# jc-bao/gym-xarm

Measured on AMD Instinct MI355X. Metric: env steps/sec (whole node), XarmPDPickAndPlace-v0, higher is better.
Workload: dtype f32

## Files before the change

### gym_xarm_amd/build.py

```python
import os
import shutil
import subprocess
import sys

HERE = os.path.dirname(os.path.abspath(__file__))
CSRC = os.path.join(HERE, "csrc")
LIB = os.path.join(CSRC, "libxarm_hip.so")
UNITS = ["xarm_hip.hip", "xarm_k_pnp.hip", "xarm_k_pnp_coop.hip", "xarm_k_reach.hip", "xarm_k_handover.hip", "xarm_k_handover_coop.hip",
         "xarm_k_handover2.hip", "xarm_k_stack.hip", "xarm_k_rearrange.hip", "xarm_k_render.hip", "xarm_k_her.hip", "xarm_k_norm.hip"]
HEADERS = ["xarm_dev.h", "xarm_core.h", "xarm7_pd_model.h", "xarm_reach_core.h", "xarm7_reach_model.h", "xarm_handover_core.h", "xarm_handover2_core.h",
           "xarm_stack_core.h", "xarm_rearrange_core.h", "xarm_coop_core.h", "xarm_reach_coop_core.h", "xarm_handover_coop_core.h", "xarm_render_core.h",
           "xarm_render_model.h", "xarm_her_core.h", "xarm_norm_core.h"]
SOURCES = UNITS + HEADERS
UNIT_FLAGS = {"xarm_k_handover_coop.hip": ["-ffp-contract=on", "-DXC_SWEEP_COPY"], "xarm_k_norm.hip": ["-ffp-contract=off"]}
_SCHED = [] if os.environ.get("XARM_SCHED", "ilp") == "default" else ["-mllvm", "-amdgpu-sched-strategy=iterative-ilp"]
HIPCC_FLAGS = ["--offload-arch=gfx950", "-O3", "-std=c++17", "-fPIC", "-Wno-unused-value", "-fno-slp-vectorize"] + _SCHED

def find_hipcc():
    for c in (os.environ.get("HIPCC"), shutil.which("hipcc"), "/opt/rocm/bin/hipcc"):
        if c and os.path.exists(c):
            return c
    raise RuntimeError("hipcc not found (need ROCm); set HIPCC=/path/to/hipcc")


def stale():
    if not os.path.exists(LIB):
        return True
    deps = [os.path.join(CSRC, s) for s in SOURCES] + [os.path.join(os.path.dirname(HERE), "include", "xarm_hip.h")]
    t = os.path.getmtime(LIB)
    return any(os.path.getmtime(d) > t for d in deps if os.path.exists(d))


def _compile(args):
    cmd, verbose = args
    if verbose:
        print(" ".join(cmd), flush=True)
    subprocess.check_call(cmd)


def build(force=False, verbose=True, extra_flags=(), lib=LIB, jobs=None):
    from concurrent.futures import ThreadPoolExecutor
    for g in ("gen_model_header.py", "gen_render_header.py"):
        gen = os.path.join(os.path.dirname(HERE), "tools", g)
        if os.path.exists(gen):
            subprocess.check_call([sys.executable, gen], stdout=subprocess.DEVNULL)
    if not force and lib == LIB and not stale():
        return lib
    hipcc = find_hipcc()
    objdir = os.path.join(CSRC, "build" if lib == LIB else "build_" + os.path.splitext(os.path.basename(lib))[0])
    os.makedirs(objdir, exist_ok=True)
    objs, jobs_l = [], []
    for u in UNITS:
        o = os.path.join(objdir, os.path.splitext(u)[0] + ".o")
        objs.append(o)
        jobs_l.append(([hipcc] + HIPCC_FLAGS + UNIT_FLAGS.get(u, []) + list(extra_flags) + ["-c", "-o", o, os.path.join(CSRC, u)], verbose))
    with ThreadPoolExecutor(jobs or min(len(UNITS), os.cpu_count() or 1)) as ex:
        list(ex.map(_compile, jobs_l))
    _compile(([hipcc, "--offload-arch=gfx950", "-shared", "-fPIC", "-o", lib] + objs, verbose))
    return lib


def build_example(verbose=True):
    root = os.path.dirname(HERE)
    src, out = os.path.join(root, "examples", "abi_step_loop.c"), os.path.join(root, "examples", "abi_step_loop")
    if not os.path.exists(src):
        return None
    if os.path.exists(out) and os.path.getmtime(out) >= max(os.path.getmtime(src), os.path.getmtime(os.path.join(root, "include", "xarm_hip.h"))):
        return out
    rocm = os.environ.get("ROCM_PATH", "/opt/rocm")
    cmd = ["gcc", "-O2", "-std=c11", "-I", os.path.join(root, "include"), "-I", os.path.join(rocm, "include"), src,
           "-L", CSRC, "-lxarm_hip", "-L", os.path.join(rocm, "lib"), "-lamdhip64",
           "-Wl,-rpath,$ORIGIN/../gym_xarm_amd/csrc", "-Wl,-rpath," + os.path.join(rocm, "lib"), "-o", out]
    if verbose:
        print(" ".join(cmd), flush=True)
    subprocess.check_call(cmd)
    return out


if __name__ == "__main__":
    build(force="--force" in sys.argv)
    print(LIB)
```

### gym_xarm_amd/csrc/xarm_coop_core.h

```cpp
#pragma once
#include "xarm_core.h"

namespace xc {
using xk::V3; using xk::mk; using xk::dot; using xk::cross; using xk::symmul; using xk::tri; using xk::symi;
using xk::EnvState; using xk::EnvCfg; using xk::NTS; using xk::NP; using xk::clampT; using xk::xabs; using xk::xsqrt;
using xk::LDS_S; using xk::LDS_T;

constexpr int GL = 16;
constexpr int NT = 3 * NTS;
constexpr int NA1 = 14;
constexpr int NF = 3 * NP;
constexpr int NLA = 7;
constexpr int C0_T = 0, C0_F = NT, C0_N = NT + NF;
constexpr int C1_A = 0, C1_L = NA1, C1_F = NA1 + NLA, C1_N = NA1 + NLA + NF;
constexpr int C2_T = 0, C2_A = NT, C2_L = NT + NA1, C2_F = NT + NA1 + NLA, C2_N = NT + NA1 + NLA + NF;

#if defined(__HIPCC__) && !defined(XARM_HOST_BUILD)
constexpr int LVN = 1;
struct Grp { int l; };
XARM_HD int lane_of(const Grp &G, int) { return G.l; }
template <int CTRL> XARM_HD float dpp(float x) {
    return __builtin_bit_cast(float, __builtin_amdgcn_update_dpp(0, __builtin_bit_cast(int, x), CTRL, 0xf, 0xf, true));
}
#else
// ... 59 lines not shown
#endif
template <int L, typename T> XARM_HD T lv_get(LV<T> x) { return lv_bcast<L>(x).v[0]; }
#if defined(__HIPCC__) && !defined(XARM_HOST_BUILD)
XARM_HD LV<float> lv_suffix_sum(LV<float> x) {
    XC_NO_CONTRACT
    float s = x.v[0];
    s += dpp<0x101>(s);
    s += dpp<0x102>(s);
    s += dpp<0x104>(s);
    s += dpp<0x108>(s);
    LV<float> r; r.v[0] = s; return r;
}
#else
template <typename T> XARM_HD LV<T> lv_suffix_sum(LV<T> x) {
    T a[GL], b[GL];
    for (int i = 0; i < GL; i++) a[i] = x.v[i];
    for (int sh = 1; sh < GL; sh *= 2) {
        for (int i = 0; i < GL; i++) b[i] = a[i] + (i + sh < GL ? a[i + sh] : (T)0);
        for (int i = 0; i < GL; i++) a[i] = b[i];
    }
    LV<T> r; for (int i = 0; i < GL; i++) r.v[i] = a[i]; return r;
}
#endif

#if defined(__HIPCC__) && !defined(XARM_HOST_BUILD)
template <typename T> struct LV2 { xk::xf2 v; };
XARM_HD LV2<float> lv2_make(LV<float> x, LV<float> y) { LV2<float> r; r.v.x = x.v[0]; r.v.y = y.v[0]; return r; }
XARM_HD LV<float> lv2_x(LV2<float> a) { LV<float> r; r.v[0] = a.v.x; return r; }
XARM_HD LV<float> lv2_y(LV2<float> a) { LV<float> r; r.v[0] = a.v.y; return r; }
XARM_HD LV2<float> lv2_fma(LV2<float> a, LV2<float> b, LV2<float> c) { LV2<float> r; r.v = __builtin_elementwise_fma(a.v, b.v, c.v); return r; }
XARM_HD LV2<float> lv2_sub(LV2<float> a, LV2<float> b) { XC_NO_CONTRACT LV2<float> r; r.v = a.v - b.v; return r; }
XARM_HD LV2<float> lv2_mul(LV2<float> a, LV2<float> b) { XC_NO_CONTRACT LV2<float> r; r.v = a.v * b.v; return r; }
template <int L> XARM_HD void lv2_commit(const Grp &G, LV2<float> &dst, LV2<float> src) { dst.v = G.l == L ? src.v : dst.v; }
template <int L> XARM_HD LV2<float> lv2_bcast(LV2<float> x) {
    LV2<float> r;
    const long long in = __builtin_bit_cast(long long, x.v);
    const long long out = __builtin_amdgcn_update_dpp(0ll, in, 0x150 + L, 0xf, 0xf, true);
    r.v = __builtin_bit_cast(xk::xf2, out);
    return r;
}
#else
template <typename T> struct LV2 { LV<T> x, y; };
template <typename T> XARM_HD LV2<T> lv2_make(LV<T> x, LV<T> y) { LV2<T> r; r.x = x; r.y = y; return r; }
template <typename T> XARM_HD LV<T> lv2_x(LV2<T> a) { return a.x; }
template <typename T> XARM_HD LV<T> lv2_y(LV2<T> a) { return a.y; }
template <typename T> XARM_HD LV2<T> lv2_fma(LV2<T> a, LV2<T> b, LV2<T> c) { return lv2_make(lv_fma(a.x, b.x, c.x), lv_fma(a.y, b.y, c.y)); }
template <typename T> XARM_HD LV2<T> lv2_sub(LV2<T> a, LV2<T> b) { return lv2_make(lv_sub(a.x, b.x), lv_sub(a.y, b.y)); }
template <typename T> XARM_HD LV2<T> lv2_mul(LV2<T> a, LV2<T> b) { return lv2_make(lv_mul(a.x, b.x), lv_mul(a.y, b.y)); }
template <int L, typename T> XARM_HD void lv2_commit(const Grp &G, LV2<T> &dst, LV2<T> src) { lv_commit<L>(G, dst.x, src.x); lv_commit<L>(G, dst.y, src.y); }
template <int L, typename T> XARM_HD LV2<T> lv2_bcast(LV2<T> x) { return lv2_make(lv_bcast<L>(x.x), lv_bcast<L>(x.y)); }
#endif

template <typename T> XARM_HD T sel3(int k, T a, T b, T c) { return k == 0 ? a : (k == 1 ? b : c); }
template <typename T> XARM_HD T sel4(int k, T a, T b, T c, T d) { return k == 0 ? a : (k == 1 ? b : (k == 2 ? c : d)); }
template <typename T> XARM_HD V3<T> selv3(int k, V3<T> a, V3<T> b, V3<T> c) { return mk<T>(sel3(k, a.x, b.x, c.x), sel3(k, a.y, b.y, c.y), sel3(k, a.z, b.z, c.z)); }
template <typename T> XARM_HD V3<T> selv4(int k, V3<T> a, V3<T> b, V3<T> c, V3<T> d) {
    return mk<T>(sel4(k, a.x, b.x, c.x, d.x), sel4(k, a.y, b.y, c.y, d.y), sel4(k, a.z, b.z, c.z, d.z));
}

template <typename T> struct Setup {
    T Minv[45], dq[9];
    V3<T> hc1;
    V3<T> cb, vb, wb;
    T Iinv[6];
    V3<T> tr[NTS];
    T tvt[NTS], tl0[NTS];
    int tid[NTS];
    T m_vt[9], la_vt[7], la_sg[7], lf_vt[2][2], g_vt;
    LV<T> lpp[3], lpn[3], lpt1[3], lpvt, lpl0;
    bool pact[NP];
    bool pad_any, la_any;
    T pad_cfm, mu_p;
};

enum { R_J0 = 0,
       R_J1 = 6,
       R_J2A = 15,
       R_J2B = 24,
       R_J3 = 30,
       R_G = 37,
       R_L0 = 41,
       R_LO1 = 45, R_HI1 = 46,
       R_CFM = 47,
       R_N = 48 };

template <typename T> XARM_HD V3<T> tdir(int a) { return mk<T>(a == 2 ? (T)1 : (T)0, a == 1 ? (T)-1 : (T)0, a == 0 ? (T)1 : (T)0); }

template <typename T, typename Scene = xk::PnpScene>
XARM_HD void lane_rows_base(const Setup<T> &S, int l, T (&R)[R_N]) {
    const T inf = (T)3.0e38;
#pragma unroll
    for (int k = 0; k < R_N; k++) R[k] = (T)0;
    {
        const int s = l / 3, a = l - 3 * s;
        const bool own = l < NT;
        const V3<T> d = tdir<T>(a);
        const V3<T> r = selv4(s, S.tr[0], S.tr[1], S.tr[2], S.tr[3]);
        const V3<T> rd = cross(r, d);
        R[R_J0 + 0] = own ? d.x : (T)0; R[R_J0 + 1] = own ? d.y : (T)0; R[R_J0 + 2] = own ? d.z : (T)0;
        R[R_J0 + 3] = own ? rd.x : (T)0; R[R_J0 + 4] = own ? rd.y : (T)0; R[R_J0 + 5] = own ? rd.z : (T)0;
        const T vt = a == 0 ? sel4(s, S.tvt[0], S.tvt[1], S.tvt[2], S.tvt[3]) : (T)0;
        const T ju = R[R_J0 + 0] * S.vb.x + R[R_J0 + 1] * S.vb.y + R[R_J0 + 2] * S.vb.z + R[R_J0 + 3] * S.wb.x + R[R_J0 + 4] * S.wb.y + R[R_J0 + 5] * S.wb.z;
        R[R_G + 0] = own ? vt - ju : (T)0;
        R[R_L0 + 0] = (own && a == 0) ? sel4(s, S.tl0[0], S.tl0[1], S.tl0[2], S.tl0[3]) : (T)0;
    }
    {
#pragma unroll
        for (int d = 0; d < 7; d++) R[R_J1 + d] = l == d ? (T)1 : (T)0;
        R[R_J1 + 7] = (l == 7 || l == 9 || l == 13) ? (T)1 : (l == 10 ? (T)-1 : (T)0);
        R[R_J1 + 8] = (l == 8 || l == 11) ? (T)1 : ((l == 12 || l == 13) ? (T)-1 : (T)0);
        T vt = (T)0, ju = (T)0;
#pragma unroll
        for (int d = 0; d < 9; d++) { vt = l == d ? S.m_vt[d] : vt; ju += R[R_J1 + d] * S.dq[d]; }
        vt = l == 9 ? S.lf_vt[0][0] : (l == 10 ? S.lf_vt[0][1] : (l == 11 ? S.lf_vt[1][0] : (l == 12 ? S.lf_vt[1][1] : (l == 13 ? S.g_vt : vt))));
        R[R_G + 1] = l < NA1 ? vt - ju : (T)0;
        const T m_hi_arm = (T)(xm::ARM_MOTOR_FORCE * Scene::TIME_STEP), m_hi_fin = (T)(Scene::FINGER_MOTOR_FORCE * Scene::TIME_STEP);
        const T g_hi = (T)(xm::GEAR_MAX_FORCE * Scene::TIME_STEP);
        const T hi = l < 7 ? m_hi_arm : (l < 9 ? m_hi_fin : (l < 13 ? inf : (l == 13 ? g_hi : (T)0)));
        R[R_HI1] = hi;
        R[R_LO1] = (l >= 9 && l < 13) ? (T)0 : -hi;
    }
}

template <typename T, typename Lds, bool PAD, bool LA>
XARM_HD void lane_rows_extra(const Setup<T> &S, Lds lds, int l, int li, T (&R)[R_N]) {
    if (PAD) {
        const int idx = l / 3, a = l - 3 * idx;
        const bool own = l < NF;
        const int fk = idx / xm::NPAD;
        const V3<T> p = mk<T>(S.lpp[0].v[li], S.lpp[1].v[li], S.lpp[2].v[li]);
        const V3<T> n = mk<T>(S.lpn[0].v[li], S.lpn[1].v[li], S.lpn[2].v[li]);
        const V3<T> t1 = mk<T>(S.lpt1[0].v[li], S.lpt1[1].v[li], S.lpt1[2].v[li]);
        const V3<T> t2 = cross(n, t1);
        const V3<T> d = selv3(a, n, t1, t2);
        const V3<T> mo = cross(p, d);
        const V3<T> af = S.hc1 * (fk == 0 ? (T)1 : (T)-1);
        const T wf = dot(af, d);
        T ju = (T)0;
#pragma unroll
        for (int i = 0; i < 7; i++) {
            const T j = lds[LDS_S + i * 6 + 0] * mo.x + lds[LDS_S + i * 6 + 1] * mo.y + lds[LDS_S + i * 6 + 2] * mo.z +
                        lds[LDS_S + i * 6 + 3] * d.x + lds[LDS_S + i * 6 + 4] * d.y + lds[LDS_S + i * 6 + 5] * d.z;
            R[R_J2A + i] = own ? j : (T)0;
            ju += R[R_J2A + i] * S.dq[i];
        }
        R[R_J2A + 7] = (own && fk == 0) ? wf : (T)0;
        R[R_J2A + 8] = (own && fk == 1) ? wf : (T)0;
        ju += R[R_J2A + 7] * S.dq[7] + R[R_J2A + 8] * S.dq[8];
        const V3<T> rb = p - S.cb;
        const V3<T> rd = cross(rb, d);
        R[R_J2B + 0] = own ? -d.x : (T)0; R[R_J2B + 1] = own ? -d.y : (T)0; R[R_J2B + 2] = own ? -d.z : (T)0;
        R[R_J2B + 3] = own ? -rd.x : (T)0; R[R_J2B + 4] = own ? -rd.y : (T)0; R[R_J2B + 5] = own ? -rd.z : (T)0;
        ju += R[R_J2B + 0] * S.vb.x + R[R_J2B + 1] * S.vb.y + R[R_J2B + 2] * S.vb.z + R[R_J2B + 3] * S.wb.x + R[R_J2B + 4] * S.wb.y + R[R_J2B + 5] * S.wb.z;
        const T vt = a == 0 ? S.lpvt.v[li] : (T)0;
        R[R_G + 2] = own ? vt - ju : (T)0;
        R[R_L0 + 2] = (own && a == 0) ? S.lpl0.v[li] : (T)0;
        R[R_CFM] = (own && a == 0) ? S.pad_cfm : (T)0;
    }
    if (LA) {
        T vt = (T)0, ju = (T)0;
#pragma unroll
        for (int d = 0; d < 7; d++) {
            R[R_J3 + d] = l == d ? S.la_sg[d] : (T)0;
            vt = l == d ? S.la_vt[d] : vt;
            ju += R[R_J3 + d] * S.dq[d];
        }
        R[R_G + 3] = l < NLA ? vt - ju : (T)0;
    }
}

template <typename T> XARM_HD void arm_row_B(const Setup<T> &S, int r, T (&B)[9]) {
#pragma unroll
    for (int d = 0; d < 9; d++) {
        if (r < 9) B[d] = S.Minv[symi(d, r)];
        else if (r == 9) B[d] = S.Minv[symi(d, 7)];
        else if (r == 10) B[d] = -S.Minv[symi(d, 7)];
        else if (r == 11) B[d] = S.Minv[symi(d, 8)];
        else if (r == 12) B[d] = -S.Minv[symi(d, 8)];
        else if (r == 13) B[d] = S.Minv[symi(d, 7)] - S.Minv[symi(d, 8)];
        else B[d] = S.la_sg[r - NA1] * S.Minv[symi(d, r - NA1)];
    }
}
template <typename T, typename Scene = xk::PnpScene>
XARM_HD void lane_delassus_base(const Setup<T> &S, int l, const T (&R)[R_N], T (&nA0)[C0_N], T (&nA1)[C1_N], T (&invd)[4]) {
    const T imb = (T)(1.0 / Scene::OBJ_MASS);
#pragma unroll
    for (int k = 0; k < 4; k++) invd[k] = (T)0;
    T diag0 = (T)1, diag1 = (T)1;
    bool act0 = false;
#pragma unroll
    for (int s = 0; s < NTS; s++)
#pragma unroll
        for (int a = 0; a < 3; a++) {
            const int r = 3 * s + a;
            const V3<T> d = tdir<T>(a);
            const V3<T> bl = d * imb, ba = symmul(S.Iinv, cross(S.tr[s], d));
            const T a0 = R[R_J0 + 0] * bl.x + R[R_J0 + 1] * bl.y + R[R_J0 + 2] * bl.z + R[R_J0 + 3] * ba.x + R[R_J0 + 4] * ba.y + R[R_J0 + 5] * ba.z;
            nA0[C0_T + r] = -a0;
            diag0 = l == r ? a0 : diag0;
            act0 = l == r ? S.tid[s] >= 0 : act0;
        }
    invd[0] = act0 ? (T)1 / diag0 : (T)0;
#pragma unroll
    for (int r = 0; r < NA1; r++) {
        T B[9];
        arm_row_B(S, r, B);
        T a1 = (T)0;
#pragma unroll
        for (int d = 0; d < 9; d++) a1 += R[R_J1 + d] * B[d];
        nA1[C1_A + r] = -a1;
        diag1 = l == r ? a1 : diag1;
    }
    invd[1] = l < NA1 ? (T)1 / diag1 : (T)0;
}
template <typename T, bool PAD, bool LA, typename Scene = xk::PnpScene>
XARM_HD void lane_delassus_extra(const Setup<T> &S, int l, const T (&R)[R_N], T (&nA1)[C1_N], T (&nA2)[C2_N], T (&nA3)[C1_N], T (&invd)[4]) {
    const T imb = (T)(1.0 / Scene::OBJ_MASS);
    T diag3 = (T)1;
    bool act3 = false;
    if (PAD) {
#pragma unroll
        for (int s = 0; s < NTS; s++)
#pragma unroll
            for (int a = 0; a < 3; a++) {
                const int r = 3 * s + a;
                const V3<T> d = tdir<T>(a);
                const V3<T> bl = d * imb, ba = symmul(S.Iinv, cross(S.tr[s], d));
                nA2[C2_T + r] = -(R[R_J2B + 0] * bl.x + R[R_J2B + 1] * bl.y + R[R_J2B + 2] * bl.z + R[R_J2B + 3] * ba.x + R[R_J2B + 4] * ba.y + R[R_J2B + 5] * ba.z);
            }
    }
#pragma unroll
    for (int r = 0; r < NA1 + NLA; r++) {
        if (!LA && r >= NA1) continue;
        T B[9];
        arm_row_B(S, r, B);
        T a1 = (T)0, a2 = (T)0, a3 = (T)0;
#pragma unroll
        for (int d = 0; d < 9; d++) {
            if (r >= NA1) a1 += R[R_J1 + d] * B[d];
            if (PAD) a2 += R[R_J2A + d] * B[d];
            if (LA && d < 7) a3 += R[R_J3 + d] * B[d];
        }
        const int c1 = r < NA1 ? C1_A + r : C1_L + (r - NA1);
        if (r >= NA1) nA1[c1] = -a1;
        if (PAD) nA2[(r < NA1 ? C2_A + r : C2_L + (r - NA1))] = -a2;
        if (LA) nA3[c1] = -a3;
        if (r >= NA1) { diag3 = l == r - NA1 ? a3 : diag3; act3 = l == r - NA1 ? S.la_sg[r - NA1] != (T)0 : act3; }
    }
    if (LA) invd[3] = act3 ? (T)1 / diag3 : (T)0;
}

template <typename T> struct Sweep {
    LV<T> g[4], lam[4], invd[4];
    LV<T> lo1, hi1;
    LV<T> nA0[C0_N], nA1[C1_N], nA2[C2_N], nA3[C1_N];
};

template <typename T, typename Scene = xk::PnpScene>
XARM_HD void pad_minv_jt(const Setup<T> &S, const LV<T> (&J)[R_G], LV<T> (&Ba)[9], LV<T> (&Bb)[6]) {
    const T imb = (T)(1.0 / Scene::OBJ_MASS);
#pragma unroll
    for (int q = 0; q < 9; q++) {
        LV<T> s = lv_scale(J[R_J2A + 0], S.Minv[symi(q, 0)]);
#pragma unroll
        for (int i = 1; i < 9; i++) s = lv_fmas(J[R_J2A + i], S.Minv[symi(q, i)], s);
        Ba[q] = s;
    }
#pragma unroll
    for (int d = 0; d < 3; d++) Bb[d] = lv_scale(J[R_J2B + d], imb);
    Bb[3] = lv_fmas(J[R_J2B + 5], S.Iinv[2], lv_fmas(J[R_J2B + 4], S.Iinv[1], lv_scale(J[R_J2B + 3], S.Iinv[0])));
    Bb[4] = lv_fmas(J[R_J2B + 5], S.Iinv[4], lv_fmas(J[R_J2B + 4], S.Iinv[3], lv_scale(J[R_J2B + 3], S.Iinv[1])));
    Bb[5] = lv_fmas(J[R_J2B + 5], S.Iinv[5], lv_fmas(J[R_J2B + 4], S.Iinv[4], lv_scale(J[R_J2B + 3], S.Iinv[2])));
}
template <typename T, bool LA, typename Scene = xk::PnpScene>
XARM_HD void pad_columns(const Grp &G, const Setup<T> &S, const LV<T> (&J)[R_G], LV<T> cfm, Sweep<T> &W, const bool (&padw)[NP]) {
    LV<T> Ba[9], Bb[6];
    pad_minv_jt<T, Scene>(S, J, Ba, Bb);
#define XC_PAD_COL(r)                                                                                        \
    if (padw[(r) / 3]) {                                                                                     \
        LV<T> ca[9], cb[6];                                                                                  \
        _Pragma("unroll") for (int q = 0; q < 9; q++) ca[q] = lv_bcast<r>(Ba[q]);                            \
        _Pragma("unroll") for (int d = 0; d < 6; d++) cb[d] = lv_bcast<r>(Bb[d]);                            \
        LV<T> a0 = lv_mul(J[R_J0], cb[0]), a1 = lv_mul(J[R_J1], ca[0]), a2 = lv_mul(J[R_J2A], ca[0]);        \
        _Pragma("unroll") for (int d = 1; d < 6; d++) a0 = lv_fma(J[R_J0 + d], cb[d], a0);                   \
        _Pragma("unroll") for (int q = 1; q < 9; q++) { a1 = lv_fma(J[R_J1 + q], ca[q], a1); a2 = lv_fma(J[R_J2A + q], ca[q], a2); } \
        _Pragma("unroll") for (int d = 0; d < 6; d++) a2 = lv_fma(J[R_J2B + d], cb[d], a2);                  \
        LV<T> diag = a2;                                                                                     \
        lv_commit<r>(G, diag, lv_add(a2, cfm));  \
        W.nA0[C0_F + r] = lv_neg(a0);                                                                        \
        W.nA1[C1_F + r] = lv_neg(a1);                                                                        \
        W.nA2[C2_F + r] = lv_neg(diag);                                                                      \
        if (LA) {                                                                                            \
            LV<T> a3 = lv_mul(J[R_J3], ca[0]);                                                               \
            _Pragma("unroll") for (int q = 1; q < 7; q++) a3 = lv_fma(J[R_J3 + q], ca[q], a3);               \
            W.nA3[C1_F + r] = lv_neg(a3);                                                                    \
        }                                                                                                    \
        lv_commit<r>(G, W.invd[2], lv_rcp_if(diag, S.pact[(r) / 3]));                                        \
    }
    XC_PAD_COL(0) XC_PAD_COL(1) XC_PAD_COL(2) XC_PAD_COL(3) XC_PAD_COL(4) XC_PAD_COL(5)
    XC_PAD_COL(6) XC_PAD_COL(7) XC_PAD_COL(8) XC_PAD_COL(9) XC_PAD_COL(10) XC_PAD_COL(11)
#undef XC_PAD_COL
}

#if defined(XC_SWEEP_ITERS) && !defined(XARM_SWEEP_VARIANT)
#define XARM_SWEEP_VARIANT XC_SWEEP_ITERS
#endif
#ifndef XC_SWEEP_ITERS
#define XC_SWEEP_ITERS xm::NUM_ITERATIONS
#endif
template <typename T, bool PAD, bool LA>
XARM_HD void sweep_all(const Grp &G, Sweep<T> &W, T mu_t, T mu_p, const bool (&padw)[NP]) {
    LV2<T> lam01 = lv2_make(W.lam[0], W.lam[1]);
    const LV2<T> invd01 = lv2_make(W.invd[0], W.invd[1]), zero2 = lv2_make(lv_fill((T)0), lv_fill((T)0));
    LV2<T> c01 = lv2_fma(lv2_make(W.g[0], W.g[1]), invd01, lam01);
    LV2<T> A01[NA1], AF01[NF];
#define XC_COL01(i)                                                                                          \
    A01[i] = lv2_mul(lv2_make((i) < NT ? W.nA0[C0_T + (i)] : lv_fill((T)0), W.nA1[C1_A + (i)]), invd01);    \
    lv2_commit<i>(G, A01[i], zero2);
    XC_COL01(0) XC_COL01(1) XC_COL01(2) XC_COL01(3) XC_COL01(4) XC_COL01(5) XC_COL01(6) XC_COL01(7) XC_COL01(8) XC_COL01(9)
    XC_COL01(10) XC_COL01(11) XC_COL01(12) XC_COL01(13)
#undef XC_COL01
    LV<T> AL1[7];
    if (LA) {
#pragma unroll
        for (int i = 0; i < 7; i++) AL1[i] = lv_mul(W.nA1[C1_L + i], W.invd[1]);
    }
    LV<T> c2 = lv_fill((T)0), c3 = lv_fill((T)0);
    if (PAD) {
        c2 = lv_fma(W.g[2], W.invd[2], W.lam[2]);
#pragma unroll
        for (int i = 0; i < NT; i++) W.nA2[C2_T + i] = lv_mul(W.nA2[C2_T + i], W.invd[2]);
#pragma unroll
        for (int i = 0; i < NA1; i++) W.nA2[C2_A + i] = lv_mul(W.nA2[C2_A + i], W.invd[2]);
        if (LA) {
#pragma unroll
            for (int i = 0; i < 7; i++) W.nA2[C2_L + i] = lv_mul(W.nA2[C2_L + i], W.invd[2]);
        }
#define XC_COLF(r)                                                                                           \
        if (padw[(r) / 3]) {                                                                                 \
            AF01[r] = lv2_mul(lv2_make(W.nA0[C0_F + r], W.nA1[C1_F + r]), invd01);                           \
            W.nA2[C2_F + r] = lv_mul(W.nA2[C2_F + r], W.invd[2]);                                            \
            lv_commit<r>(G, W.nA2[C2_F + r], lv_fill((T)0));                                                 \
            if (LA) W.nA3[C1_F + r] = lv_mul(W.nA3[C1_F + r], W.invd[3]);                                    \
        }
        XC_COLF(0) XC_COLF(1) XC_COLF(2) XC_COLF(3) XC_COLF(4) XC_COLF(5) XC_COLF(6) XC_COLF(7) XC_COLF(8) XC_COLF(9) XC_COLF(10) XC_COLF(11)
#undef XC_COLF
    }
    if (LA) {
        c3 = lv_fma(W.g[3], W.invd[3], W.lam[3]);
#pragma unroll
        for (int i = 0; i < NA1; i++) W.nA3[C1_A + i] = lv_mul(W.nA3[C1_A + i], W.invd[3]);
#define XC_COLL(i)                                                                                           \
        W.nA3[C1_L + i] = lv_mul(W.nA3[C1_L + i], W.invd[3]);                                                \
        lv_commit<i>(G, W.nA3[C1_L + i], lv_fill((T)0));
        XC_COLL(0) XC_COLL(1) XC_COLL(2) XC_COLL(3) XC_COLL(4) XC_COLL(5) XC_COLL(6)
#undef XC_COLL
    }
    const LV<T> mu_tv = lv_fill_vgpr(mu_t), mu_pv = lv_fill(mu_p);
#ifdef XC_SWEEP_COPY
    constexpr int NL_SETS = 1;
#else
    constexpr int NL_SETS = 2;
#endif
    LV2<T> NL[NL_SETS][NA1];
#pragma unroll
    for (int i = 0; i < NA1; i++) NL[0][i] = lam01;
    bool law[NLA];
#define XC_LAW(i) law[i] = LA && XARM_ANY_X(lv_get<i>(W.invd[3]) != (T)0);
    XC_LAW(0) XC_LAW(1) XC_LAW(2) XC_LAW(3) XC_LAW(4) XC_LAW(5) XC_LAW(6)
#undef XC_LAW
#define XC_PAIR(i, RD, WR)                                                                                   \
        {                                                                                                    \
            LV<T> nx = lv2_x(c01);                                                                           \
            if ((i) % 3 == 0 || (i) >= NT) nx = lv_max0(nx);                                                 \
            else nx = lv_med3(nx, lv_neg(lim), lim);                                                         \
            const LV2<T> nl = lv2_make(nx, lv_med3(lv2_y(c01), W.lo1, W.hi1));                               \
            const LV2<T> dl = lv2_sub(nl, NL[RD][i]);                                                        \
            NL[WR][i] = nl;                                     \
            if ((i) % 3 == 0 && (i) < NT) lim = lv_mul(lv_bcast<i>(nx), mu_tv);  \
            const LV2<T> b = lv2_bcast<i>(dl);                                                               \
            c01 = lv2_fma(A01[i], b, c01);                                                                   \
            if (PAD) {                                                                                       \
                if ((i) < NT) c2 = lv_fma(W.nA2[C2_T + (i)], lv2_x(b), c2);                                  \
                c2 = lv_fma(W.nA2[C2_A + (i)], lv2_y(b), c2);                                                \
            }                                                                                                \
            if (LA) c3 = lv_fma(W.nA3[C1_A + (i)], lv2_y(b), c3);                                            \
        }
#define XC_L_ROW(i)                                                                                          \
        if (law[i]) {                                                                                        \
            const LV<T> nl = lv_max0(c3);                                                                    \
            const LV<T> dl = lv_sub(nl, W.lam[3]);                                                           \
            lv_commit<i>(G, W.lam[3], nl);                                                                   \
            const LV<T> b = lv_bcast<i>(dl);                                                                 \
            c01 = lv2_make(lv2_x(c01), lv_fma(AL1[i], b, lv2_y(c01)));                                       \
            if (PAD) c2 = lv_fma(W.nA2[C2_L + i], b, c2);                                                    \
            c3 = lv_fma(W.nA3[C1_L + i], b, c3);                                                             \
        }
#define XC_F_ROW(p, a)                                                                                       \
        {                                                                                                    \
            LV<T> nl;                                                                                        \
            if ((a) == 0) nl = lv_max0(c2);                                                                  \
            else {                                                                                           \
                const LV<T> flim = lv_mul(lv_bcast<3 * p>(W.lam[2]), mu_pv);                                 \
                nl = lv_med3(c2, lv_neg(flim), flim);                                                        \
            }                                                                                                \
            const LV<T> dl = lv_sub(nl, W.lam[2]);                                                           \
            lv_commit<3 * p + a>(G, W.lam[2], nl);                                                           \
            const LV<T> b = lv_bcast<3 * p + a>(dl);                                                         \
            c01 = lv2_fma(AF01[3 * p + a], lv2_make(b, b), c01);                                             \
            c2 = lv_fma(W.nA2[C2_F + 3 * p + a], b, c2);                                                     \
            if (LA) c3 = lv_fma(W.nA3[C1_F + 3 * p + a], b, c3);                                             \
        }
#define XC_F_PAD(p) if (padw[p]) { XC_F_ROW(p, 0) XC_F_ROW(p, 1) XC_F_ROW(p, 2) }
#define XC_SWEEP(RD, WR)                                                                                     \
    {                                                                                                        \
        LV<T> lim = lv_fill((T)0);                                                                           \
        XC_PAIR(0, RD, WR) XC_PAIR(1, RD, WR) XC_PAIR(2, RD, WR) XC_PAIR(3, RD, WR) XC_PAIR(4, RD, WR)       \
        XC_PAIR(5, RD, WR) XC_PAIR(6, RD, WR) XC_PAIR(7, RD, WR) XC_PAIR(8, RD, WR)                          \
        if (LA) { XC_L_ROW(0) XC_L_ROW(1) XC_L_ROW(2) XC_L_ROW(3) XC_L_ROW(4) XC_L_ROW(5) XC_L_ROW(6) }      \
        XC_PAIR(9, RD, WR) XC_PAIR(10, RD, WR) XC_PAIR(11, RD, WR) XC_PAIR(12, RD, WR) XC_PAIR(13, RD, WR)   \
        if (PAD) { XC_F_PAD(0) XC_F_PAD(1) XC_F_PAD(2) XC_F_PAD(3) }                                         \
    }
    constexpr int NSW = XC_SWEEP_ITERS;
#ifdef XC_SWEEP_COPY
    constexpr int LAST = 0;
#pragma unroll 1
    for (int it = 0; it < NSW; it++) XC_SWEEP(0, 0)
#else
    constexpr int LAST = NSW & 1;
#pragma unroll 1
    for (int it = 0; it + 1 < NSW; it += 2) {
        XC_SWEEP(0, 1)
        XC_SWEEP(1, 0)
    }
    if (NSW & 1) XC_SWEEP(0, 1)
#endif
#undef XC_SWEEP
#undef XC_PAIR
#undef XC_L_ROW
#undef XC_F_ROW
#undef XC_F_PAD
#define XC_KEEP(i) lv2_commit<i>(G, lam01, NL[LAST][i]);
    XC_KEEP(0) XC_KEEP(1) XC_KEEP(2) XC_KEEP(3) XC_KEEP(4) XC_KEEP(5) XC_KEEP(6) XC_KEEP(7) XC_KEEP(8) XC_KEEP(9)
    XC_KEEP(10) XC_KEEP(11) XC_KEEP(12) XC_KEEP(13)
#undef XC_KEEP
    W.lam[0] = lv2_x(lam01);
    W.lam[1] = lv2_y(lam01);
}

template <typename T, bool PAD, bool LA> XARM_HD void apply_warm_start(Sweep<T> &W, const bool (&padw)[NP]) {
#define XC_WS_T(s)                                                                                           \
    {                                                                                                        \
        const LV<T> b = lv_bcast<3 * s>(W.lam[0]);                                                           \
        W.g[0] = lv_fma(W.nA0[C0_T + 3 * s], b, W.g[0]);                                                    \
        if (PAD) W.g[2] = lv_fma(W.nA2[C2_T + 3 * s], b, W.g[2]);                                           \
    }
    XC_WS_T(0) XC_WS_T(1) XC_WS_T(2) XC_WS_T(3)
    if (PAD) {
#define XC_WS_F(p)                                                                                           \
    if (padw[p]) {                                                                                                     \
        const LV<T> b = lv_bcast<3 * p>(W.lam[2]);                                                           \
        W.g[0] = lv_fma(W.nA0[C0_F + 3 * p], b, W.g[0]);                                                    \
        W.g[1] = lv_fma(W.nA1[C1_F + 3 * p], b, W.g[1]);                                                    \
        W.g[2] = lv_fma(W.nA2[C2_F + 3 * p], b, W.g[2]);                                                    \
        if (LA) W.g[3] = lv_fma(W.nA3[C1_F + 3 * p], b, W.g[3]);                                            \
    }
        XC_WS_F(0) XC_WS_F(1) XC_WS_F(2) XC_WS_F(3)
    }
#undef XC_WS_T
#undef XC_WS_F
}

template <typename T> struct ArmLane { LV<T> mass, com[3], inertia[6], damping; };
template <typename T> XARM_HD ArmLane<T> arm_lane_consts(const Grp &G) {
    ArmLane<T> C;
    XC_LANES {
        const int l = lane_of(G, i_);
        T m = (T)0, dmp = (T)0, c[3] = {(T)0, (T)0, (T)0}, in[6] = {(T)0, (T)0, (T)0, (T)0, (T)0, (T)0};
#pragma unroll
        for (int b = 0; b < 9; b++) {
            m = l == b ? (T)xm::MASS[b] : m;
            dmp = l == b ? (T)xm::DAMPING[b] : dmp;
#pragma unroll
            for (int k = 0; k < 3; k++) c[k] = l == b ? (T)xm::COM[b][k] : c[k];
#pragma unroll
            for (int k = 0; k < 6; k++) in[k] = l == b ? (T)xm::INERTIA[b][k] : in[k];
        }
        C.mass.v[i_] = m; C.damping.v[i_] = dmp;
#pragma unroll
        for (int k = 0; k < 3; k++) C.com[k].v[i_] = c[k];
#pragma unroll
        for (int k = 0; k < 6; k++) C.inertia[k].v[i_] = in[k];
    }
    return C;
}

template <typename T, typename Lds, typename Scene = xk::PnpScene>
XARM_HD void arm_dynamics_coop(const Grp &G, const ArmLane<T> &C, const T (&q_in)[9], const T (&qd_in)[9], const T dt, Lds lds, xk::ArmDyn<T> &A, const int arm = 0) {
    using xk::SV; using xk::RBI; using xk::Frame;
    SV<T> S[7];
    Frame<T> f = Scene::template base_frame<T>(arm);
    SV<T> vel, acc;
    vel.w = mk<T>(0, 0, 0); vel.v = mk<T>(0, 0, 0);
    acc.w = mk<T>(0, 0, 0); acc.v = mk<T>(0, 0, (T)xm::GRAVITY);
    LV<T> cap[24], capqd = lv_fill((T)0);
#pragma unroll
    for (int k = 0; k < 24; k++) cap[k] = lv_fill((T)0);
#define XC_CAPTURE(i, fr, vv, aa, qdv)                                                                       \
    {                                                                                                        \
        const T vals[24] = {fr.c0.x, fr.c0.y, fr.c0.z, fr.c1.x, fr.c1.y, fr.c1.z, fr.c2.x, fr.c2.y, fr.c2.z, fr.o.x, fr.o.y, fr.o.z, \
                            vv.w.x, vv.w.y, vv.w.z, vv.v.x, vv.v.y, vv.v.z, aa.w.x, aa.w.y, aa.w.z, aa.v.x, aa.v.y, aa.v.z}; \
        _Pragma("unroll") for (int k = 0; k < 24; k++) lv_commit<i>(G, cap[k], lv_fill(vals[k]));            \
        lv_commit<i>(G, capqd, lv_fill(qdv));                                                                \
    }
#define XC_CHAIN(i)                                                                                          \
    {                                                                                                        \
        xk::fk_advance(f, i, q_in[i]);                                                                       \
        S[i].w = f.c2;                                                                                       \
        S[i].v = cross(f.o, f.c2);                                                                           \
        const T qd = qd_in[i];                                                                               \
        acc.w = acc.w + cross(vel.w, S[i].w) * qd;                                                           \
        acc.v = acc.v + (cross(vel.w, S[i].v) + cross(vel.v, S[i].w)) * qd;                                  \
        vel.w = vel.w + S[i].w * qd;                                                                         \
        vel.v = vel.v + S[i].v * qd;                                                                         \
        XC_CAPTURE(i, f, vel, acc, qd)                                                                       \
    }
    XC_CHAIN(0) XC_CHAIN(1) XC_CHAIN(2) XC_CHAIN(3) XC_CHAIN(4) XC_CHAIN(5) XC_CHAIN(6)
#undef XC_CHAIN
    const V3<T> hc0 = f.c0, hc1 = f.c1, hc2 = f.c2, ho = f.o;
    A.hc0 = hc0; A.hc1 = hc1; A.hc2 = hc2;
#define XC_FINGER(k)                                                                                         \
    {                                                                                                        \
        const T sg = k == 0 ? (T)1 : (T)-1;                                                                  \
        const V3<T> af = hc1 * sg;                                                                           \
        A.fo[k] = ho + hc2 * (T)xm::FINGER_Z + af * q_in[7 + k];                                             \
        const T qd = qd_in[7 + k];                                                                           \
        SV<T> v = vel, a = acc;                                                                              \
        a.v = a.v + cross(vel.w, af) * qd;                                                                   \
        v.v = v.v + af * qd;                                                                                 \
        Frame<T> ff; ff.c0 = hc0; ff.c1 = hc1; ff.c2 = hc2; ff.o = A.fo[k];                                  \
        XC_CAPTURE(7 + k, ff, v, a, qd)                                                                      \
    }
    XC_FINGER(0) XC_FINGER(1)
#undef XC_FINGER
#undef XC_CAPTURE
    LV<T> body[16], comp[16], Mrow[9], taul;
    XC_LANES {
        const int l = lane_of(G, i_);
        const V3<T> c0 = mk<T>(cap[0].v[i_], cap[1].v[i_], cap[2].v[i_]), c1 = mk<T>(cap[3].v[i_], cap[4].v[i_], cap[5].v[i_]),
                    c2 = mk<T>(cap[6].v[i_], cap[7].v[i_], cap[8].v[i_]), o = mk<T>(cap[9].v[i_], cap[10].v[i_], cap[11].v[i_]);
        SV<T> v, a;
        v.w = mk<T>(cap[12].v[i_], cap[13].v[i_], cap[14].v[i_]); v.v = mk<T>(cap[15].v[i_], cap[16].v[i_], cap[17].v[i_]);
        a.w = mk<T>(cap[18].v[i_], cap[19].v[i_], cap[20].v[i_]); a.v = mk<T>(cap[21].v[i_], cap[22].v[i_], cap[23].v[i_]);
        const T m = C.mass.v[i_];
        const V3<T> c = o + c0 * C.com[0].v[i_] + c1 * C.com[1].v[i_] + c2 * C.com[2].v[i_];
        const T ixx = C.inertia[0].v[i_], ixy = C.inertia[1].v[i_], ixz = C.inertia[2].v[i_], iyy = C.inertia[3].v[i_],
                iyz = C.inertia[4].v[i_], izz = C.inertia[5].v[i_];
        const V3<T> m0 = c0 * ixx + c1 * ixy + c2 * ixz, m1 = c0 * ixy + c1 * iyy + c2 * iyz, m2 = c0 * ixz + c1 * iyz + c2 * izz;
        const T cc = dot(c, c);
        RBI<T> I;
        I.m = m;
        I.h = c * m;
        I.I[0] = m0.x * c0.x + m1.x * c1.x + m2.x * c2.x + m * (cc - c.x * c.x);
        I.I[1] = m0.x * c0.y + m1.x * c1.y + m2.x * c2.y - m * c.x * c.y;
        I.I[2] = m0.x * c0.z + m1.x * c1.z + m2.x * c2.z - m * c.x * c.z;
        I.I[3] = m0.y * c0.y + m1.y * c1.y + m2.y * c2.y + m * (cc - c.y * c.y);
        I.I[4] = m0.y * c0.z + m1.y * c1.z + m2.y * c2.z - m * c.y * c.z;
        I.I[5] = m0.z * c0.z + m1.z * c1.z + m2.z * c2.z + m * (cc - c.z * c.z);
        const SV<T> Iv = xk::rbi_mul(I, v), Ia = xk::rbi_mul(I, a);
        SV<T> fbias;
        fbias.w = Ia.w + cross(v.w, Iv.w) + cross(v.v, Iv.v);
        fbias.v = Ia.v + cross(v.w, Iv.v);
        const T vals[16] = {I.m, I.h.x, I.h.y, I.h.z, I.I[0], I.I[1], I.I[2], I.I[3], I.I[4], I.I[5],
                            fbias.w.x, fbias.w.y, fbias.w.z, fbias.v.x, fbias.v.y, fbias.v.z};
#pragma unroll
        for (int k = 0; k < 16; k++) body[k].v[i_] = l < 9 ? vals[k] : (T)0;
    }
#pragma unroll
    for (int k = 0; k < 16; k++) comp[k] = lv_suffix_sum(body[k]);
    XC_LANES {
        const int l = lane_of(G, i_);
        const bool fin = l >= 7;
        RBI<T> Ic;
        SV<T> fc, Sl;
        const LV<T> *src = comp;
        Ic.m = fin ? body[0].v[i_] : src[0].v[i_];
        Ic.h = mk<T>(fin ? body[1].v[i_] : src[1].v[i_], fin ? body[2].v[i_] : src[2].v[i_], fin ? body[3].v[i_] : src[3].v[i_]);
#pragma unroll
        for (int k = 0; k < 6; k++) Ic.I[k] = fin ? body[4 + k].v[i_] : src[4 + k].v[i_];
        fc.w = mk<T>(fin ? body[10].v[i_] : src[10].v[i_], fin ? body[11].v[i_] : src[11].v[i_], fin ? body[12].v[i_] : src[12].v[i_]);
        fc.v = mk<T>(fin ? body[13].v[i_] : src[13].v[i_], fin ? body[14].v[i_] : src[14].v[i_], fin ? body[15].v[i_] : src[15].v[i_]);
        const V3<T> c1 = mk<T>(cap[3].v[i_], cap[4].v[i_], cap[5].v[i_]), c2 = mk<T>(cap[6].v[i_], cap[7].v[i_], cap[8].v[i_]),
                    o = mk<T>(cap[9].v[i_], cap[10].v[i_], cap[11].v[i_]);
        const V3<T> ax = c1 * (l == 8 ? (T)-1 : (T)1);
        Sl.w = fin ? mk<T>(0, 0, 0) : c2;
        Sl.v = fin ? ax : cross(o, c2);
        const SV<T> F = xk::rbi_mul(Ic, Sl);
#pragma unroll
        for (int i = 0; i < 7; i++) Mrow[i].v[i_] = xk::sdot(S[i], F);
        Mrow[7].v[i_] = l == 7 ? dot(ax, F.v) : (T)0;
        Mrow[8].v[i_] = l == 8 ? dot(ax, F.v) : (T)0;
        taul.v[i_] = -xk::sdot(Sl, fc) - C.damping.v[i_] * capqd.v[i_];
    }
    T M[45], tau[9];
#define XC_ROW(r)                                                                                            \
    {                                                                                                        \
        _Pragma("unroll") for (int c = 0; c <= r; c++) M[tri(r, c)] = lv_get<r>(Mrow[c]);                    \
        tau[r] = lv_get<r>(taul);                                                                            \
    }
    XC_ROW(0) XC_ROW(1) XC_ROW(2) XC_ROW(3) XC_ROW(4) XC_ROW(5) XC_ROW(6) XC_ROW(7) XC_ROW(8)
#undef XC_ROW
    T (&Minv)[45] = A.Minv;
    {
        T rd[9];
#pragma unroll
        for (int c = 0; c < 9; c++) {
#pragma unroll
            for (int r = c; r < 9; r++) {
                T s = M[tri(r, c)];
#pragma unroll
                for (int k = 0; k < c; k++) s -= M[tri(r, k)] * M[tri(c, k)];
                if (r == c) { M[tri(c, c)] = xsqrt(s); rd[c] = (T)1 / M[tri(c, c)]; }
                else M[tri(r, c)] = s * rd[c];
            }
        }
        T Li[45];
#pragma unroll
        for (int c = 0; c < 9; c++) {
            Li[tri(c, c)] = rd[c];
#pragma unroll
            for (int r = c + 1; r < 9; r++) {
                T s = (T)0;
#pragma unroll
                for (int k = c; k < r; k++) s -= M[tri(r, k)] * Li[tri(k, c)];
                Li[tri(r, c)] = s * rd[r];
            }
        }
#pragma unroll
        for (int r = 0; r < 9; r++)
#pragma unroll
            for (int c = 0; c <= r; c++) {
                T s = (T)0;
#pragma unroll
                for (int k = r; k < 9; k++) s += Li[tri(k, r)] * Li[tri(k, c)];
                Minv[tri(r, c)] = s;
            }
    }
#pragma unroll
    for (int r = 0; r < 9; r++) {
        T s = (T)0;
#pragma unroll
        for (int c = 0; c < 9; c++) s += Minv[symi(r, c)] * tau[c];
        A.dq[r] = qd_in[r] + dt * s;
    }
#pragma unroll
    for (int i = 0; i < 7; i++) {
        lds[LDS_S + i * 6 + 0] = S[i].w.x; lds[LDS_S + i * 6 + 1] = S[i].w.y; lds[LDS_S + i * 6 + 2] = S[i].w.z;
        lds[LDS_S + i * 6 + 3] = S[i].v.x; lds[LDS_S + i * 6 + 4] = S[i].v.y; lds[LDS_S + i * 6 + 5] = S[i].v.z;
    }
    XARM_LDS_FENCE();
}

template <typename T, typename Lds, typename Scene = xk::PnpScene>
XARM_HD void substep_setup(const Grp &G, const ArmLane<T> &C, EnvState<T> &st, const T (&qt)[9], const T dt, Lds lds, Setup<T> &S, const int arm = 0) {
    const T idt = (T)1 / dt;
    xk::ArmDyn<T> AD;
    arm_dynamics_coop<T, Lds, Scene>(G, C, st.q, st.qd, dt, lds, AD, arm);
#pragma unroll
    for (int k = 0; k < 45; k++) S.Minv[k] = AD.Minv[k];
#pragma unroll
    for (int k = 0; k < 9; k++) S.dq[k] = AD.dq[k];
    S.hc1 = AD.hc1;
    const V3<T> hc0 = AD.hc0, hc1 = AD.hc1, hc2 = AD.hc2;
    V3<T> b0, b1, b2;
    {
        const T x = st.bq[0], y = st.bq[1], z = st.bq[2], w = st.bq[3];
        b0 = mk<T>((T)1 - (T)2 * (y * y + z * z), (T)2 * (x * y + z * w), (T)2 * (x * z - y * w));
        b1 = mk<T>((T)2 * (x * y - z * w), (T)1 - (T)2 * (x * x + z * z), (T)2 * (y * z + x * w));
        b2 = mk<T>((T)2 * (x * z + y * w), (T)2 * (y * z - x * w), (T)1 - (T)2 * (x * x + y * y));
    }
    const V3<T> cb = mk<T>(st.bp[0], st.bp[1], st.bp[2]);
    S.cb = cb;
    const T hx = (T)Scene::OBJ_HX, hy = (T)Scene::OBJ_HY, hz = (T)Scene::OBJ_HZ;
    const T Ibx = (T)(Scene::OBJ_MASS / 3.0 * (Scene::OBJ_HY * Scene::OBJ_HY + Scene::OBJ_HZ * Scene::OBJ_HZ));
    const T Iby = (T)(Scene::OBJ_MASS / 3.0 * (Scene::OBJ_HX * Scene::OBJ_HX + Scene::OBJ_HZ * Scene::OBJ_HZ));
    const T Ibz = (T)(Scene::OBJ_MASS / 3.0 * (Scene::OBJ_HX * Scene::OBJ_HX + Scene::OBJ_HY * Scene::OBJ_HY));
    {
        const T ix = (T)1 / Ibx, iy = (T)1 / Iby, iz = (T)1 / Ibz;
        S.Iinv[0] = b0.x * b0.x * ix + b1.x * b1.x * iy + b2.x * b2.x * iz;
        S.Iinv[1] = b0.x * b0.y * ix + b1.x * b1.y * iy + b2.x * b2.y * iz;
        S.Iinv[2] = b0.x * b0.z * ix + b1.x * b1.z * iy + b2.x * b2.z * iz;
        S.Iinv[3] = b0.y * b0.y * ix + b1.y * b1.y * iy + b2.y * b2.y * iz;
        S.Iinv[4] = b0.y * b0.z * ix + b1.y * b1.z * iy + b2.y * b2.z * iz;
        S.Iinv[5] = b0.z * b0.z * ix + b1.z * b1.z * iy + b2.z * b2.z * iz;
    }
    V3<T> vb = mk<T>(st.bv[0], st.bv[1], st.bv[2]), wb = mk<T>(st.bw[0], st.bw[1], st.bw[2]);
    {
        const V3<T> wl = mk<T>(dot(b0, wb), dot(b1, wb), dot(b2, wb));
        const V3<T> iw = mk<T>(Ibx * wl.x, Iby * wl.y, Ibz * wl.z);
        const V3<T> f = cross(wl, iw) * dt;
        const T J00 = Ibx, J01 = dt * (-wl.z * Iby + iw.z), J02 = dt * (wl.y * Ibz - iw.y);
        const T J10 = dt * (wl.z * Ibx - iw.z), J11 = Iby, J12 = dt * (-wl.x * Ibz + iw.x);
        const T J20 = dt * (-wl.y * Ibx + iw.y), J21 = dt * (wl.x * Iby - iw.x), J22 = Ibz;
        const T c00 = J11 * J22 - J12 * J21, c01 = J12 * J20 - J10 * J22, c02 = J10 * J21 - J11 * J20;
        const T id = (T)1 / (J00 * c00 + J01 * c01 + J02 * c02);
        const V3<T> x = mk<T>((f.x * c00 + f.y * (J02 * J21 - J01 * J22) + f.z * (J01 * J12 - J02 * J11)) * id,
                              (f.x * c01 + f.y * (J00 * J22 - J02 * J20) + f.z * (J02 * J10 - J00 * J12)) * id,
                              (f.x * c02 + f.y * (J01 * J20 - J00 * J21) + f.z * (J00 * J11 - J01 * J10)) * id);
        const V3<T> wn = wl - x;
        wb = b0 * wn.x + b1 * wn.y + b2 * wn.z;
        vb.z -= dt * (T)xm::GRAVITY;
        vb = vb * (T)Scene::LIN_DAMP_FACTOR;
        wb = wb * (T)Scene::ANG_DAMP_FACTOR;
    }
    S.vb = vb; S.wb = wb;
#pragma unroll
    for (int s = 0; s < NTS; s++) { S.tr[s] = mk<T>(0, 0, 0); S.tvt[s] = (T)0; S.tl0[s] = (T)0; S.tid[s] = -1; }
    {
        int cnt = 0;
#pragma unroll
        for (int i = 0; i < 8; i++) {
            const V3<T> r = b0 * ((i & 1) ? hx : -hx) + b1 * ((i & 2) ? hy : -hy) + b2 * ((i & 4) ? hz : -hz);
            const V3<T> p = cb + r;
            T hsup;
            const bool sup = Scene::template support<T>(p, hsup);
            const T dist = p.z - hsup;
            const bool act = dist < (T)xm::SOLVER_MARGIN && sup && cnt < NTS;
            const T vt = dist < (T)0 ? -(T)xm::CONTACT_ERP * dist * idt : -dist * idt;
            const T l0 = (T)xm::WARMSTART * st.lam_t[i];
#pragma unroll
            for (int s = 0; s < NTS; s++) {
                const bool put = act && cnt == s;
                S.tr[s] = xk::selv(put, r, S.tr[s]);
                S.tvt[s] = put ? vt : S.tvt[s];
                S.tl0[s] = put ? l0 : S.tl0[s];
                S.tid[s] = put ? i : S.tid[s];
            }
            cnt += act ? 1 : 0;
        }
        if constexpr (Scene::HAS_STAND) {
            V3<T> sp[4];
            T sd[4];
            Scene::template stand_points<T>(st.goal, cb, b0, b1, b2, sp, sd);
#pragma unroll
            for (int v = 0; v < 4; v++) {
                const T dist = sd[v];
                const bool act = dist < (T)xm::SOLVER_MARGIN && dist > (T)Scene::STAND_MIN_GAP && cnt < NTS;
                const V3<T> r = sp[v] - cb;
// ... 308 lines not shown
```

Baseline: 16.44 million.

## Keep pad friction impulses in per-row registers and specialize all-pads-active sweep

For the padded, non-lookahead coop sweep (PnP coop), the pad friction lambdas are now held in per-row register arrays (NLF) instead of being committed back to a lane each row, and are written back once after the loop. A separate loop instantiation covers the case where all four pads are active, so the per-pad branches disappear there. Friction limits are now computed from the freshly updated normal impulse rather than the previous one, which changes the Gauss-Seidel numerics slightly. The handover coop unit keeps the old behaviour through a V1 flag. The cost is more register pressure and a duplicated loop body.

```diff
diff --git a/gym_xarm_amd/build.py b/gym_xarm_amd/build.py
--- a/gym_xarm_amd/build.py
+++ b/gym_xarm_amd/build.py
@@ -12,7 +12,7 @@
            "xarm_stack_core.h", "xarm_rearrange_core.h", "xarm_coop_core.h", "xarm_reach_coop_core.h", "xarm_handover_coop_core.h", "xarm_render_core.h",
            "xarm_render_model.h", "xarm_her_core.h", "xarm_norm_core.h"]
 SOURCES = UNITS + HEADERS
-UNIT_FLAGS = {"xarm_k_handover_coop.hip": ["-ffp-contract=on", "-DXC_SWEEP_COPY"], "xarm_k_norm.hip": ["-ffp-contract=off"]}
+UNIT_FLAGS = {"xarm_k_handover_coop.hip": ["-ffp-contract=on", "-DXC_SWEEP_COPY", "-DXC_PAD_ROWS_V1"], "xarm_k_norm.hip": ["-ffp-contract=off"]}
 _SCHED = [] if os.environ.get("XARM_SCHED", "ilp") == "default" else ["-mllvm", "-amdgpu-sched-strategy=iterative-ilp"]
 HIPCC_FLAGS = ["--offload-arch=gfx950", "-O3", "-std=c++17", "-fPIC", "-Wno-unused-value", "-fno-slp-vectorize"] + _SCHED
 
diff --git a/gym_xarm_amd/csrc/xarm_coop_core.h b/gym_xarm_amd/csrc/xarm_coop_core.h
--- a/gym_xarm_amd/csrc/xarm_coop_core.h
+++ b/gym_xarm_amd/csrc/xarm_coop_core.h
@@ -385,6 +385,11 @@
 #undef XC_PAD_COL
 }
 
+#ifndef XC_ROW_CENSUS
+#define XC_ROW_CENSUS(pad, la, padw, law)
+#elif !defined(XARM_HOST_BUILD)
+#error "XC_ROW_CENSUS is a host-build hook"
+#endif
 #if defined(XC_SWEEP_ITERS) && !defined(XARM_SWEEP_VARIANT)
 #define XARM_SWEEP_VARIANT XC_SWEEP_ITERS
 #endif
@@ -408,6 +413,11 @@
 #pragma unroll
         for (int i = 0; i < 7; i++) AL1[i] = lv_mul(W.nA1[C1_L + i], W.invd[1]);
     }
+#ifdef XC_PAD_ROWS_V1
+    constexpr bool FRESH_FLIM = false, FCF = false;
+#else
+    constexpr bool FRESH_FLIM = true, FCF = PAD && !LA;
+#endif
     LV<T> c2 = lv_fill((T)0), c3 = lv_fill((T)0);
     if (PAD) {
         c2 = lv_fma(W.g[2], W.invd[2], W.lam[2]);
@@ -448,10 +458,16 @@
     LV2<T> NL[NL_SETS][NA1];
 #pragma unroll
     for (int i = 0; i < NA1; i++) NL[0][i] = lam01;
+    LV<T> NLF[NL_SETS][NF];
+    if (FCF) {
+#pragma unroll
+        for (int r = 0; r < NF; r++) NLF[0][r] = W.lam[2];
+    }
     bool law[NLA];
 #define XC_LAW(i) law[i] = LA && XARM_ANY_X(lv_get<i>(W.invd[3]) != (T)0);
     XC_LAW(0) XC_LAW(1) XC_LAW(2) XC_LAW(3) XC_LAW(4) XC_LAW(5) XC_LAW(6)
 #undef XC_LAW
+    XC_ROW_CENSUS(PAD, LA, padw, law)
 #define XC_PAIR(i, RD, WR)                                                                                   \
         {                                                                                                    \
             LV<T> nx = lv2_x(c01);                                                                           \
@@ -479,45 +495,51 @@
             if (PAD) c2 = lv_fma(W.nA2[C2_L + i], b, c2);                                                    \
             c3 = lv_fma(W.nA3[C1_L + i], b, c3);                                                             \
         }
-#define XC_F_ROW(p, a)                                                                                       \
+#define XC_F_ROW(p, a, RD, WR)                                                                               \
         {                                                                                                    \
             LV<T> nl;                                                                                        \
-            if ((a) == 0) nl = lv_max0(c2);                                                                  \
-            else {                                                                                           \
-                const LV<T> flim = lv_mul(lv_bcast<3 * p>(W.lam[2]), mu_pv);                                 \
+            if ((a) == 0) {                                                                                  \
+                nl = lv_max0(c2);                                                                            \
+                if (FRESH_FLIM) flim = lv_mul(lv_bcast<3 * p>(nl), mu_pv);                                   \
+            } else {                                                                                         \
+                if (!FRESH_FLIM) flim = lv_mul(lv_bcast<3 * p>(W.lam[2]), mu_pv);                            \
                 nl = lv_med3(c2, lv_neg(flim), flim);                                                        \
             }                                                                                                \
-            const LV<T> dl = lv_sub(nl, W.lam[2]);                                                           \
-            lv_commit<3 * p + a>(G, W.lam[2], nl);                                                           \
+            const LV<T> dl = lv_sub(nl, FCF ? NLF[RD][3 * p + a] : W.lam[2]);                                \
+            if (FCF) NLF[WR][3 * p + a] = nl;                                                                \
+            else lv_commit<3 * p + a>(G, W.lam[2], nl);                                                      \
             const LV<T> b = lv_bcast<3 * p + a>(dl);                                                         \
             c01 = lv2_fma(AF01[3 * p + a], lv2_make(b, b), c01);                                             \
             c2 = lv_fma(W.nA2[C2_F + 3 * p + a], b, c2);                                                     \
             if (LA) c3 = lv_fma(W.nA3[C1_F + 3 * p + a], b, c3);                                             \
         }
-#define XC_F_PAD(p) if (padw[p]) { XC_F_ROW(p, 0) XC_F_ROW(p, 1) XC_F_ROW(p, 2) }
-#define XC_SWEEP(RD, WR)                                                                                     \
+#define XC_F_PAD(p, RD, WR, ALLP) if (ALLP || padw[p]) { LV<T> flim = lv_fill((T)0); XC_F_ROW(p, 0, RD, WR) XC_F_ROW(p, 1, RD, WR) XC_F_ROW(p, 2, RD, WR) }
+#define XC_SWEEP(RD, WR, ALLP)                                                                               \
     {                                                                                                        \
         LV<T> lim = lv_fill((T)0);                                                                           \
         XC_PAIR(0, RD, WR) XC_PAIR(1, RD, WR) XC_PAIR(2, RD, WR) XC_PAIR(3, RD, WR) XC_PAIR(4, RD, WR)       \
         XC_PAIR(5, RD, WR) XC_PAIR(6, RD, WR) XC_PAIR(7, RD, WR) XC_PAIR(8, RD, WR)                          \
         if (LA) { XC_L_ROW(0) XC_L_ROW(1) XC_L_ROW(2) XC_L_ROW(3) XC_L_ROW(4) XC_L_ROW(5) XC_L_ROW(6) }      \
         XC_PAIR(9, RD, WR) XC_PAIR(10, RD, WR) XC_PAIR(11, RD, WR) XC_PAIR(12, RD, WR) XC_PAIR(13, RD, WR)   \
-        if (PAD) { XC_F_PAD(0) XC_F_PAD(1) XC_F_PAD(2) XC_F_PAD(3) }                                         \
+        if (PAD) { XC_F_PAD(0, RD, WR, ALLP) XC_F_PAD(1, RD, WR, ALLP) XC_F_PAD(2, RD, WR, ALLP) XC_F_PAD(3, RD, WR, ALLP) } \
     }
     constexpr int NSW = XC_SWEEP_ITERS;
 #ifdef XC_SWEEP_COPY
     constexpr int LAST = 0;
-#pragma unroll 1
-    for (int it = 0; it < NSW; it++) XC_SWEEP(0, 0)
+#define XC_LOOP(ALLP)                                                                                        \
+    _Pragma("unroll 1") for (int it = 0; it < NSW; it++) XC_SWEEP(0, 0, ALLP)
 #else
     constexpr int LAST = NSW & 1;
-#pragma unroll 1
-    for (int it = 0; it + 1 < NSW; it += 2) {
-        XC_SWEEP(0, 1)
-        XC_SWEEP(1, 0)
-    }
-    if (NSW & 1) XC_SWEEP(0, 1)
-#endif
+#define XC_LOOP(ALLP)                                                                                        \
+    _Pragma("unroll 1") for (int it = 0; it + 1 < NSW; it += 2) {                                            \
+        XC_SWEEP(0, 1, ALLP)                                                                                 \
+        XC_SWEEP(1, 0, ALLP)                                                                                 \
+    }                                                                                                        \
+    if (NSW & 1) XC_SWEEP(0, 1, ALLP)
+#endif
+    if (FCF && padw[0] && padw[1] && padw[2] && padw[3]) { XC_LOOP(true) }
+    else { XC_LOOP(false) }
+#undef XC_LOOP
 #undef XC_SWEEP
 #undef XC_PAIR
 #undef XC_L_ROW
@@ -527,6 +549,12 @@
     XC_KEEP(0) XC_KEEP(1) XC_KEEP(2) XC_KEEP(3) XC_KEEP(4) XC_KEEP(5) XC_KEEP(6) XC_KEEP(7) XC_KEEP(8) XC_KEEP(9)
     XC_KEEP(10) XC_KEEP(11) XC_KEEP(12) XC_KEEP(13)
 #undef XC_KEEP
+    if (FCF) {
+#define XC_KEEPF(r) if (padw[(r) / 3]) lv_commit<r>(G, W.lam[2], NLF[LAST][r]);
+        XC_KEEPF(0) XC_KEEPF(1) XC_KEEPF(2) XC_KEEPF(3) XC_KEEPF(4) XC_KEEPF(5) XC_KEEPF(6) XC_KEEPF(7) XC_KEEPF(8) XC_KEEPF(9)
+        XC_KEEPF(10) XC_KEEPF(11)
+#undef XC_KEEPF
+    }
     W.lam[0] = lv2_x(lam01);
     W.lam[1] = lv2_y(lam01);
 }
```

After: 17.53 million, median of 6. 6.6% higher.
